# intellerce/controlanimate

Measured on AMD Instinct MI355X. Metric: frames_per_sec, higher is better.
Workload: dtype fp16

## Files before the change

controlanimate_amd/_build.py:

```python
from __future__ import annotations

import os
import subprocess
import sys
from concurrent.futures import ThreadPoolExecutor

CSRC = os.path.join(os.path.dirname(os.path.abspath(__file__)), "csrc")
LIB = os.path.join(CSRC, "libcontrolanimate_hip.so")
SOURCES = ["ca_gemm.hip", "ca_gemm_pp.hip", "ca_gemm_ar.hip", "ca_norm.hip", "ca_attention.hip", "ca_elementwise.hip", "ca_upscale.hip", "ca_color.hip", "ca_canny.hip"]
HEADERS = ["ca_common.h", "ca_gemm_core.h", "ca_gemm_pp2.h", "ca_gemm_wres.h", "ca_gemm_ps.h", "ca_gemm_pq.h", "ca_gemm_ar.h", "ca_ff_fused.h", "ca_attn_out.h", "ca_tattn_fused.h", "ca_xattn_fused.h", "ca_gemm_seq.h", "ca_conv_wino.h", os.path.join("..", "..", "include", "controlanimate_hip.h")]
FLAGS = ["--offload-arch=gfx950", "-O3", "-std=c++17", "-fPIC", "-Wall", "-Wno-unused-function",
         "-mllvm", "-amdgpu-mfma-vgpr-form"]


EXTRA = {"ca_attention.hip": ["-fno-honor-nans"],
         "ca_color.hip": ["-ffp-contract=off"]}


def _extra_env_flags() -> list:
    return os.environ.get("CA_HIPCC_FLAGS", "").split()


def _hipcc() -> str:
    for cand in (os.environ.get("HIPCC"), "/opt/rocm/bin/hipcc", "hipcc"):
        if cand and (os.path.sep not in cand or os.path.exists(cand)):
            return cand
    raise RuntimeError("hipcc not found")


def _stale(out: str, deps: list[str]) -> bool:
    if not os.path.exists(out):
        return True
    t = os.path.getmtime(out)
    return any(os.path.getmtime(d) > t for d in deps)


LIB_EXP = os.path.join(CSRC, "libcontrolanimate_hip_exp.so")
LIB_STAMPS = os.path.join(CSRC, "libcontrolanimate_hip_stamps.so")


def build(force: bool = False, verbose: bool = True, experiments: bool = False, stamps: bool = False) -> str:
    hipcc = _hipcc()
# ... 35 lines not shown
```

controlanimate_amd/_capi.py:

```python
from __future__ import annotations

import ctypes as C
import os

_HERE = os.path.dirname(os.path.abspath(__file__))
LIB_PATH = os.environ.get("CA_HIP_LIB") or os.path.join(_HERE, "csrc", "libcontrolanimate_hip.so")

CA_BF16, CA_F16 = 0, 1
CA_F32 = 2
CA_ACT_NONE, CA_ACT_SILU = 0, 1
ABI_VERSION = 16


class CAHipUnavailable(RuntimeError):
    pass


class CAHipError(RuntimeError):
    pass


class GemmArgs(C.Structure):
    _fields_ = [
        ("a", C.c_void_p), ("a2", C.c_void_p), ("w", C.c_void_p), ("c", C.c_void_p),
# ... 155 lines not shown
    "ca_latents_to_nhwc": (C.c_int, [C.c_void_p, C.c_void_p, C.c_int32, C.c_int32, C.c_int32, C.c_int32, C.c_int32,
                                      C.c_int32, C.c_int32, C.c_float, C.c_int32, C.c_void_p]),
    "ca_nhwc_to_ncfhw_f32": (C.c_int, [C.c_void_p, C.c_void_p, C.c_int32, C.c_int32, C.c_int32, C.c_int32, C.c_int32,
                                        C.c_int32, C.c_int32, C.c_int32, C.c_void_p]),
    "ca_ncfhw_to_nhwc": (C.c_int, [C.c_void_p, C.c_int32, C.POINTER(C.c_int64), C.c_void_p, C.c_int32, C.c_int32,
                                    C.c_int32, C.c_int32, C.c_int32, C.c_int32, C.c_int32, C.c_void_p]),
    "ca_cfg_scheduler_step": (C.c_int, [C.c_void_p, C.c_int32, C.c_int32, C.c_float, C.c_void_p, C.c_void_p,
                                         C.c_void_p, C.c_void_p, C.c_int32, C.c_int32, C.c_int32, C.c_int32,
                                         C.POINTER(C.c_float), C.c_float, C.c_void_p]),
    "ca_lincomb": (C.c_int, [C.c_void_p, C.POINTER(C.c_void_p), C.POINTER(C.c_float), C.c_int32, C.c_int64, C.c_void_p]),
    "ca_conv3x3_narrow": (C.c_int, [C.POINTER(ConvNarrowArgs), C.c_void_p]),
    "ca_conv3x3_narrow_plan_name": (C.c_int, [C.POINTER(ConvNarrowArgs), C.c_char_p, C.c_int32]),
    "ca_rgb8_to_nhwc": (C.c_int, [C.c_void_p, C.c_void_p, C.c_int32, C.c_int32, C.c_int32, C.c_int32, C.c_void_p]),
    "ca_resize_lanczos4_u8": (C.c_int, [C.c_void_p, C.c_void_p, C.c_int32, C.c_int32, C.c_int32, C.c_int32, C.c_int32,
                                         C.c_void_p, C.c_void_p, C.c_void_p, C.c_void_p, C.c_void_p]),
    "ca_color_match_workspace_bytes": (C.c_int64, [C.c_int32, C.c_int64]),
    "ca_hist_u8x3": (C.c_int, [C.c_void_p, C.c_void_p, C.c_int32, C.c_int64, C.c_void_p]),
    "ca_color_moments_f64": (C.c_int, [C.c_void_p, C.c_void_p, C.c_void_p, C.c_void_p, C.c_int32, C.c_int64, C.c_void_p, C.c_int64, C.c_void_p]),
    "ca_color_transform_f64": (C.c_int, [C.c_void_p, C.c_void_p, C.c_void_p, C.c_void_p, C.c_void_p, C.c_void_p, C.c_int32, C.c_int64, C.c_void_p]),
    "ca_sort_f64_segments": (C.c_int, [C.c_void_p, C.c_void_p, C.c_int32, C.c_int64, C.c_void_p, C.c_int64, C.c_void_p]),
    "ca_color_rank_map_f64": (C.c_int, [C.c_void_p, C.c_void_p, C.c_void_p, C.c_void_p, C.c_void_p, C.c_void_p, C.c_int32, C.c_int64,
                                         C.c_void_p, C.c_int64, C.c_void_p]),
    "ca_color_finish_u8": (C.c_int, [C.c_void_p, C.c_void_p, C.c_int32, C.c_int64, C.c_int32, C.c_void_p, C.c_int64, C.c_void_p]),
    "ca_canny_workspace_bytes": (C.c_int64, [C.c_int32, C.c_int32, C.c_int32]),
    "ca_canny_tile_w": (C.c_int32, []),
    "ca_canny_tile_h": (C.c_int32, []),
    "ca_canny_classify": (C.c_int, [C.c_void_p, C.c_int32, C.c_int32, C.c_int32, C.c_int32, C.c_int32, C.c_int32, C.c_void_p, C.c_int64, C.c_void_p]),
    "ca_canny_link": (C.c_int, [C.c_int32, C.c_int32, C.c_int32, C.c_void_p, C.c_int64, C.c_void_p]),
    "ca_canny_link_stage": (C.c_int, [C.c_int32, C.c_int32, C.c_int32, C.c_void_p, C.c_int64, C.c_int32, C.c_void_p]),
    "ca_canny_emit": (C.c_int, [C.c_int32, C.c_int32, C.c_int32, C.c_void_p, C.c_int64, C.c_void_p, C.c_void_p, C.c_int32, C.c_int32, C.c_void_p]),
    "ca_conv_up2_phase_supported": (C.c_int, [C.POINTER(ConvArgs)]),
    "ca_conv_up2_phase": (C.c_int, [C.POINTER(ConvArgs), C.c_void_p]),
    "ca_conv_up2_phase_plan_name": (C.c_int, [C.POINTER(ConvArgs), C.c_char_p, C.c_int32]),
}

_lib = None


def lib() -> C.CDLL:
    global _lib
    if _lib is not None:
        return _lib
    import torch
    if not os.path.exists(LIB_PATH):
        raise CAHipUnavailable(
            f"{LIB_PATH} is missing: the HIP extension is not built. Run "
            "`python -m controlanimate_amd._build` (needs hipcc); there is no CPU fallback.")
    try:
        handle = C.CDLL(LIB_PATH)
    except OSError as e:
        raise CAHipUnavailable(f"cannot load {LIB_PATH}: {e}") from e
    for name, (res, args) in SYMBOLS.items():
        fn = getattr(handle, name)
        fn.restype = res
        fn.argtypes = args
    if handle.ca_abi_version() != ABI_VERSION:
        raise CAHipUnavailable(f"ABI mismatch: library {handle.ca_abi_version()} vs binding {ABI_VERSION}; rebuild")
    _lib = handle
    return handle


def check(rc: int, what: str) -> None:
    if rc != 0:
        msg = lib().ca_last_error()
        raise CAHipError(f"{what} failed with code {rc}: {msg.decode() if msg else ''}")
```

controlanimate_amd/context.py:

```python
from __future__ import annotations

from dataclasses import dataclass, field
from typing import Optional

import torch


@dataclass
class ExecCtx:
    b: int
    f: int
    dtype: torch.dtype
    temb: torch.Tensor
    emb_groups: int
    ehs: Optional[torch.Tensor] = None
    frames_per_kv: int = 1
    kv_mod: int = 0
    gn_frames_per_stat: int = 1
    cache: dict = field(default_factory=dict)

    @property
    def images(self) -> int:
        return self.b * self.f

    def rows_per_emb_group(self, h: int, w: int) -> int:
        return self.images // self.emb_groups * h * w


class Dispatch:
    gemm_ar = True
    ff_fused = True
    tattn_fused = True
    xattn_fused = True
    attn_out_fused = True
    xattn_ip_fused = True
    conv_winograd = True
    gn_winograd = True
    conv_up2_phase = True
    ln_row_sums = True
    repeat_kernel = True
    ln_fold = True
    cfg_shared = True
    cn_cfg_dedup = True
    controlnet_streams = 2


dispatch = Dispatch()
```

controlanimate_amd/controlnet.py:

```python
from __future__ import annotations

import dataclasses
from collections import OrderedDict

from typing import List, Optional, Sequence, Tuple, Union

import torch
from torch import nn

from . import kernels as K
from .context import ExecCtx
from .layers import HipConv1x1, HipConv3x3
from .unet import FrozenConfig, HipModelMixin, TimestepEmbedding, Timesteps
from .unet_blocks import UNetMidBlock3DCrossAttn, get_down_block


class ControlNetConditioningEmbedding(nn.Module):
    def __init__(self, conditioning_embedding_channels: int, conditioning_channels: int = 3,
                 block_out_channels: Tuple[int, ...] = (16, 32, 96, 256)):
        super().__init__()
        self.conv_in = HipConv3x3(conditioning_channels, block_out_channels[0])
        blocks = []
        for i in range(len(block_out_channels) - 1):
            blocks.append(HipConv3x3(block_out_channels[i], block_out_channels[i]))
            blocks.append(HipConv3x3(block_out_channels[i], block_out_channels[i + 1], stride=2))
        self.blocks = nn.ModuleList(blocks)
        self.conv_out = HipConv3x3(block_out_channels[-1], conditioning_embedding_channels)
        nn.init.zeros_(self.conv_out.weight)

    def pack(self, arena, dtype):
        self.conv_in.pack(arena, dtype)
        for b in self.blocks:
            b.pack(arena, dtype)
        self.conv_out.pack(arena, dtype)

    def forward(self, cond_nhwc: torch.Tensor) -> torch.Tensor:
        e = self.conv_in.run(cond_nhwc, act=K.ACT_SILU)
        for b in self.blocks:
            e = b.run(e, act=K.ACT_SILU)
        return self.conv_out.run(e)


class ControlNetModel(HipModelMixin, nn.Module):
    def __init__(self, in_channels: int = 4, conditioning_channels: int = 3, flip_sin_to_cos: bool = True, freq_shift: int = 0,
                 down_block_types: Tuple[str, ...] = ("CrossAttnDownBlock2D", "CrossAttnDownBlock2D", "CrossAttnDownBlock2D", "DownBlock2D"),
                 only_cross_attention: bool = False, block_out_channels: Tuple[int, ...] = (320, 640, 1280, 1280),
                 layers_per_block: int = 2, downsample_padding: int = 1, mid_block_scale_factor: float = 1, act_fn: str = "silu",
                 norm_num_groups: int = 32, norm_eps: float = 1e-5, cross_attention_dim: int = 768,
                 attention_head_dim: Union[int, Tuple[int, ...]] = 8, use_linear_projection: bool = False,
                 conditioning_embedding_out_channels: Tuple[int, ...] = (16, 32, 96, 256), global_pool_conditions: bool = False,
                 **unused):
        super().__init__()
        self._init_exec()
        if use_linear_projection or global_pool_conditions:
            raise NotImplementedError("not part of the SD1.5 ControlNet configuration")
        cfg = dict(locals())
        for k in ("self", "unused", "__class__"):
            cfg.pop(k, None)
        self.config = FrozenConfig(cfg)
        time_embed_dim = block_out_channels[0] * 4
        self.conv_in = HipConv3x3(in_channels, block_out_channels[0])
        self.time_proj = Timesteps(block_out_channels[0], flip_sin_to_cos, freq_shift)
        self.time_embedding = TimestepEmbedding(block_out_channels[0], time_embed_dim, act_fn=act_fn)
        self.controlnet_cond_embedding = ControlNetConditioningEmbedding(block_out_channels[0], conditioning_channels,
                                                                         conditioning_embedding_out_channels)
        self.down_blocks = nn.ModuleList([])
        self.controlnet_down_blocks = nn.ModuleList([HipConv1x1(block_out_channels[0], block_out_channels[0])])
        if isinstance(attention_head_dim, int):
            attention_head_dim = (attention_head_dim,) * len(down_block_types)
        common = dict(temb_channels=time_embed_dim, resnet_eps=norm_eps, resnet_groups=norm_num_groups,
                      cross_attention_dim=cross_attention_dim, use_inflated_groupnorm=True, use_motion_module=False)
        output_channel = block_out_channels[0]
        for i, t in enumerate(down_block_types):
            input_channel, output_channel = output_channel, block_out_channels[i]
            is_final = i == len(block_out_channels) - 1
            self.down_blocks.append(get_down_block(t, num_layers=layers_per_block, in_channels=input_channel,
                                                   out_channels=output_channel, add_downsample=not is_final,
                                                   attn_num_head_channels=attention_head_dim[i], **common))
            for _ in range(layers_per_block + (0 if is_final else 1)):
                self.controlnet_down_blocks.append(HipConv1x1(output_channel, output_channel))
        self.controlnet_mid_block = HipConv1x1(block_out_channels[-1], block_out_channels[-1])
        self.mid_block = UNetMidBlock3DCrossAttn(in_channels=block_out_channels[-1], output_scale_factor=mid_block_scale_factor,
                                                 attn_num_head_channels=attention_head_dim[-1], **common)
        for m in list(self.controlnet_down_blocks) + [self.controlnet_mid_block]:
            nn.init.zeros_(m.weight)
        self._hints: "OrderedDict[int, dict]" = OrderedDict()

    @classmethod
    def from_config(cls, config: dict, **kwargs):
        merged = {k: v for k, v in dict(config).items() if not k.startswith("_")}
        merged.update(kwargs)
        return cls(**merged)

    def hint_slot(self, controlnet_cond: Optional[torch.Tensor] = None) -> Optional[dict]:
# ... 207 lines not shown
```

controlanimate_amd/kernels.py:

```python
from __future__ import annotations

import ctypes as C
from typing import Optional

import torch

from . import _capi
from .context import dispatch
from ._capi import (AttnArgs, ConvArgs, ConvNarrowArgs, FfArgs, TattnArgs, XattnArgs, GemmArgs, GroupNormArgs, LayerNormArgs, CA_ACT_NONE,
                    CA_ACT_SILU, CA_BF16, CA_F16, check, lib)

ACT_NONE, ACT_SILU = CA_ACT_NONE, CA_ACT_SILU
ACT_QUICK_GELU, ACT_GELU = 2, 3


def dt_code(dtype: torch.dtype) -> int:
    if dtype == torch.bfloat16:
        return CA_BF16
    if dtype == torch.float16:
        return CA_F16
    raise TypeError(f"activations must be bf16 or fp16, got {dtype}")


def _stream() -> int:
# ... 200 lines not shown
        return None
    if _plan_sink is not None:
        _plan_sink.append(("xattn_ip_out128" if kv_frag_ip is not None else "xattn_out128") if w_out_frag is not None else "xattn_fused128")
    check(lib().ca_xattn_fused(C.byref(args), _stream()), "ca_xattn_fused")
    return o


def row_sums_of(t: torch.Tensor):
    return getattr(t, "_row_sums", None)


def carry_row_sums(dst: torch.Tensor, src: torch.Tensor) -> torch.Tensor:
    s = getattr(src, "_row_sums", None)
    if s is not None:
        dst._row_sums = s
    return dst


class RowStats:

    def __init__(self, x: torch.Tensor, eps: float = 1e-5, sums=None):
        self.x, self.eps, self._t, self.sums = x, float(eps), None, sums

    def tensor(self) -> torch.Tensor:
        if self._t is None:
            self._t = row_stats(self.x, self.eps)
        return self._t


def conv3x3(x: torch.Tensor, w: torch.Tensor, *, x2: Optional[torch.Tensor] = None,
            bias: Optional[torch.Tensor] = None, rowbias: Optional[torch.Tensor] = None,
            rows_per_group: int = 0, residual: Optional[torch.Tensor] = None, stride: int = 1,
            upsample: bool = False, alpha: float = 1.0, post_scale: float = 1.0, act: int = ACT_NONE,
            out_f32: bool = False, pad_asym: bool = False, w_wino: Optional[torch.Tensor] = None) -> torch.Tensor:
    _req_cuda(x, w, x2, bias, rowbias, residual, w_wino)
    assert x.dim() == 4 and x.is_contiguous() and w.dim() == 4 and w.is_contiguous()
    images, hin, win, cin1 = x.shape
    cin2 = 0
    if x2 is not None:
        assert x2.is_contiguous() and x2.shape[:3] == x.shape[:3] and x2.dtype == x.dtype
        cin2 = x2.shape[3]
    cout = w.shape[0]
    assert tuple(w.shape[1:]) == (3, 3, cin1 + cin2) and w.dtype == x.dtype
    hl, wl = (hin * 2, win * 2) if upsample else (hin, win)
    pad = 1 if pad_asym else 2
    hout, wout = (hl + pad - 3) // stride + 1, (wl + pad - 3) // stride + 1
    y = torch.empty((images, hout, wout, cout), device=x.device, dtype=torch.float32 if out_f32 else x.dtype)
    ld_res = 0
    if residual is not None:
        assert residual.dtype == x.dtype and residual.is_contiguous() and residual.numel() == images * hout * wout * cout, \
            f"residual {tuple(residual.shape)} {residual.dtype} contiguous={residual.is_contiguous()} vs output {(images, hout, wout, cout)} {x.dtype}"
        ld_res = cout
    if rowbias is not None:
        assert rowbias.dtype == torch.float32 and rowbias.dim() == 2 and rowbias.shape[1] == cout and rows_per_group > 0
    if bias is not None:
        assert bias.dtype == torch.float32 and bias.numel() == cout
    args = ConvArgs(x=_p(x), x2=_p(x2), w=_p(w), y=_p(y), bias=_p(bias), rowbias=_p(rowbias),
                    residual=_p(residual), ld_res=ld_res,
                    ld_rowbias=rowbias.stride(0) if rowbias is not None else 0, images=images, hin=hin,
                    win=win, cin1=cin1, cin2=cin2, cout=cout, stride=stride, upsample=int(upsample),
                    rows_per_group=rows_per_group, alpha=alpha, post_scale=post_scale, act=act,
                    out_f32=int(out_f32), dtype=dt_code(x.dtype), pad_asym=int(pad_asym))
    if w_wino is not None and dispatch.conv_winograd:
        assert w_wino.dtype == x.dtype and w_wino.is_contiguous() and tuple(w_wino.shape) == (16, cout, cin1 + cin2)
        args.w_wino = _p(w_wino)
    wbytes = int(lib().ca_conv3x3_workspace_bytes(C.byref(args)))
    if wbytes > 0:
        ws = torch.empty((wbytes,), device=x.device, dtype=torch.uint8)
        args.workspace, args.workspace_bytes = _p(ws), wbytes
    _record_plan(lib().ca_conv3x3_plan_name, args)
    check(lib().ca_conv3x3(C.byref(args), _stream()), "ca_conv3x3")
    return y


def _up2_args(x, w_phase, bias, residual, alpha, y=None) -> ConvArgs:
    images, hin, win, cin = x.shape
    cout = w_phase.shape[1]
    return ConvArgs(x=_p(x), w=_p(w_phase), y=_p(y) if y is not None else _p(x), bias=_p(bias), residual=_p(residual),
                    ld_res=cout if residual is not None else 0, images=images, hin=hin, win=win, cin1=cin, cin2=0, cout=cout, stride=1,
                    upsample=1, rows_per_group=0, alpha=alpha, post_scale=1.0, act=ACT_NONE, out_f32=0, dtype=dt_code(x.dtype), pad_asym=0)


def conv_up2_phase_supported(x: torch.Tensor, w_phase: torch.Tensor, *, bias: Optional[torch.Tensor] = None,
                             residual: Optional[torch.Tensor] = None, alpha: float = 1.0) -> bool:
    if x.dim() != 4 or w_phase.dim() != 5 or not x.is_contiguous() or x.dtype not in (torch.float16, torch.bfloat16):
        return False
    return bool(lib().ca_conv_up2_phase_supported(C.byref(_up2_args(x, w_phase, bias, residual, alpha))))


def conv_up2_phase(x: torch.Tensor, w_phase: torch.Tensor, *, bias: Optional[torch.Tensor] = None,
                   residual: Optional[torch.Tensor] = None, alpha: float = 1.0) -> torch.Tensor:
    _req_cuda(x, w_phase, bias, residual)
    assert x.dim() == 4 and x.is_contiguous() and w_phase.dim() == 5 and w_phase.is_contiguous() and w_phase.dtype == x.dtype
    images, hin, win, cin = x.shape
    cout = w_phase.shape[1]
# ... 473 lines not shown
```

controlanimate_amd/layers.py:

```python
from __future__ import annotations

from typing import Callable, List, Optional, Sequence, Tuple

import torch
from torch import nn

from . import kernels as K
from .context import dispatch

ALIGN = 256


class Packed:

    __slots__ = ("shape", "dtype", "fill", "offset", "t", "frag")

    def __init__(self, shape, dtype, fill):
        self.shape = tuple(int(s) for s in shape)
        self.dtype = dtype
        self.fill = fill
        self.offset = -1
        self.t: Optional[torch.Tensor] = None
        self.frag = None

# ... 120 lines not shown
        super().__init__()
        self.in_channels, self.out_channels = in_channels, out_channels
        self.weight = nn.Parameter(torch.empty(out_channels, in_channels, 1, 1))
        self.bias = nn.Parameter(torch.zeros(out_channels))
        nn.init.normal_(self.weight, std=in_channels ** -0.5)
        self.w = self.b = None

    def pack(self, arena: WeightArena, dtype):
        self.w = arena.add((self.out_channels, self.in_channels), dtype, lambda: _f32(self.weight).reshape(self.out_channels, self.in_channels))
        self.b = arena.add((self.out_channels,), torch.float32, lambda: _f32(self.bias))

    def run(self, a: torch.Tensor, **kw) -> torch.Tensor:
        return K.gemm(a, self.w.t, bias=self.b.t, **kw)


def phase_weights(w: torch.Tensor) -> torch.Tensor:
    sel = torch.tensor([[[1.0, 0.0, 0.0], [0.0, 1.0, 1.0]], [[1.0, 1.0, 0.0], [0.0, 0.0, 1.0]]], dtype=w.dtype, device=w.device)
    wp = torch.einsum("ydk,xel,oikl->yxodei", sel, sel, w)
    return wp.reshape(4, w.shape[0], 2, 2, w.shape[1]).contiguous()


class HipConv3x3(nn.Module):

    def __init__(self, in_channels: int, out_channels: int, stride: int = 1):
        super().__init__()
        self.in_channels, self.out_channels, self.stride = in_channels, out_channels, stride
        self.cin_pad = (in_channels + 7) // 8 * 8
        self.weight = nn.Parameter(torch.empty(out_channels, in_channels, 3, 3))
        self.bias = nn.Parameter(torch.zeros(out_channels))
        nn.init.normal_(self.weight, std=(9 * in_channels) ** -0.5)
        self.w = self.b = None
        self.winograd = True
        self.up2_phase = False

    def _packed_weight(self) -> torch.Tensor:
        w = _f32(self.weight).permute(0, 2, 3, 1)
        if self.cin_pad != self.in_channels:
            w = torch.nn.functional.pad(w, (0, self.cin_pad - self.in_channels))
        return w.contiguous()

    def _winograd_weight(self) -> torch.Tensor:
        g = torch.tensor([[1.0, 0.0, 0.0], [0.5, 0.5, 0.5], [0.5, -0.5, 0.5], [0.0, 0.0, 1.0]], dtype=torch.float32, device=self.weight.device)
        u = torch.einsum("xk,oikl,yl->xyoi", g, _f32(self.weight), g)
        return u.reshape(16, self.out_channels, self.in_channels).contiguous()

    def pack(self, arena: WeightArena, dtype):
        self.w = arena.add((self.out_channels, 3, 3, self.cin_pad), dtype, self._packed_weight)
        self.b = arena.add((self.out_channels,), torch.float32, lambda: _f32(self.bias))
        self.u = None
        if (dispatch.conv_winograd and self.stride == 1 and self.winograd and self.in_channels >= 640 and self.in_channels % 64 == 0
                and self.out_channels % 320 == 0):
            self.u = arena.add((16, self.out_channels, self.in_channels), dtype, self._winograd_weight)
        self.wp = None
        if dispatch.conv_up2_phase and self.up2_phase and self.stride == 1 and self.in_channels % 64 == 0 and self.out_channels % 320 == 0:
            self.wp = arena.add((4, self.out_channels, 2, 2, self.in_channels), dtype, lambda: phase_weights(_f32(self.weight)))

    def run(self, x: torch.Tensor, **kw) -> torch.Tensor:
        wp = getattr(self, "wp", None)
        if wp is not None and dispatch.conv_up2_phase and kw.get("upsample") and set(kw) <= {"upsample", "residual", "alpha"}:
            ph = {k: v for k, v in kw.items() if k != "upsample"}
            if K.conv_up2_phase_supported(x, wp.t, bias=self.b.t, **ph):
                return K.conv_up2_phase(x, wp.t, bias=self.b.t, **ph)
        u = getattr(self, "u", None)
        return K.conv3x3(x, self.w.t, bias=self.b.t, stride=self.stride, w_wino=None if u is None else u.t, **kw)


class HipGroupNorm(nn.Module):
    def __init__(self, num_groups: int, num_channels: int, eps: float = 1e-5):
        super().__init__()
        self.num_groups, self.num_channels, self.eps = num_groups, num_channels, eps
        self.weight = nn.Parameter(torch.ones(num_channels))
        self.bias = nn.Parameter(torch.zeros(num_channels))
        self.g = self.b = None

    def pack(self, arena: WeightArena, dtype):
        self.g = arena.add((self.num_channels,), torch.float32, lambda: _f32(self.weight))
        self.b = arena.add((self.num_channels,), torch.float32, lambda: _f32(self.bias))

    def run(self, x: torch.Tensor, *, x2: Optional[torch.Tensor] = None, frames_per_stat: int = 1, act: int = K.ACT_NONE):
        return K.group_norm(x, self.g.t, self.b.t, x2=x2, groups=self.num_groups, frames_per_stat=frames_per_stat,
                            eps=self.eps, act=act)


class HipLayerNorm(nn.Module):
    def __init__(self, dim: int, eps: float = 1e-5):
        super().__init__()
        self.dim, self.eps = dim, eps
        self.weight = nn.Parameter(torch.ones(dim))
        self.bias = nn.Parameter(torch.zeros(dim))
        self.g = self.b = None

    def pack(self, arena: WeightArena, dtype):
        self.g = arena.add((self.dim,), torch.float32, lambda: _f32(self.weight))
        self.b = arena.add((self.dim,), torch.float32, lambda: _f32(self.bias))

    def run(self, x: torch.Tensor, *, pos: Optional[torch.Tensor] = None, rows_per_frame: int = 1, frames: int = 1):
        return K.layer_norm(x, self.g.t, self.b.t, pos=pos, rows_per_frame=rows_per_frame, frames=frames, eps=self.eps)
# ... 62 lines not shown
```

controlanimate_amd/unet.py:

```python
from __future__ import annotations

from collections import OrderedDict

import dataclasses
import json
import os
from dataclasses import dataclass
from typing import Any, Dict, Optional, Tuple, Union

import torch
from torch import nn

from . import kernels as K
from .context import ExecCtx, dispatch
from .layers import HipGroupNorm, HipLinear, WeightArena, pack_concat_bias, pack_concat_rows
from .resnet import InflatedConv3d, InflatedGroupNorm, ResnetBlock3D
from .unet_blocks import UNetMidBlock3DCrossAttn, get_down_block, get_up_block


@dataclass
class UNet3DConditionOutput:
    sample: torch.Tensor


# ... 246 lines not shown
        class_embed_type: Optional[str] = None,
        num_class_embeds: Optional[int] = None,
        upcast_attention: bool = False,
        resnet_time_scale_shift: str = "default",
        use_inflated_groupnorm: bool = False,
        time_cond_proj_dim: Optional[int] = None,
        use_motion_module: bool = False,
        motion_module_resolutions: Tuple[int, ...] = (1, 2, 4, 8),
        motion_module_mid_block: bool = False,
        motion_module_decoder_only: bool = False,
        motion_module_type: Optional[str] = None,
        motion_module_kwargs: Optional[dict] = None,
        unet_use_cross_frame_attention: Optional[bool] = None,
        unet_use_temporal_attention: Optional[bool] = None,
        **unused,
    ):
        super().__init__()
        self._init_exec()
        if class_embed_type is not None or num_class_embeds is not None or dual_cross_attention or use_linear_projection:
            raise NotImplementedError("not part of the SD1.5 configuration the reference runs")
        if act_fn not in ("silu", "swish") or resnet_time_scale_shift != "default" or center_input_sample:
            raise NotImplementedError("SD1.5 uses silu / default time-embedding norm")
        cfg = dict(locals())
        for k in ("self", "unused", "__class__"):
            cfg.pop(k, None)
        cfg.update(unused)
        self.config = FrozenConfig(cfg)
        self.sample_size = sample_size
        self.in_channels = in_channels
        motion_module_kwargs = dict(motion_module_kwargs or {})
        time_embed_dim = block_out_channels[0] * 4

        self.conv_in = InflatedConv3d(in_channels, block_out_channels[0])
        self.time_proj = Timesteps(block_out_channels[0], flip_sin_to_cos, freq_shift)
        self.time_embedding = TimestepEmbedding(block_out_channels[0], time_embed_dim, act_fn=act_fn, cond_proj_dim=time_cond_proj_dim)

        self.down_blocks = nn.ModuleList([])
        self.up_blocks = nn.ModuleList([])
        if isinstance(attention_head_dim, int):
            attention_head_dim = (attention_head_dim,) * len(down_block_types)
        common = dict(temb_channels=time_embed_dim, resnet_eps=norm_eps, resnet_groups=norm_num_groups,
                      cross_attention_dim=cross_attention_dim, use_inflated_groupnorm=use_inflated_groupnorm,
                      motion_module_type=motion_module_type, motion_module_kwargs=motion_module_kwargs,
                      unet_use_cross_frame_attention=bool(unet_use_cross_frame_attention),
                      unet_use_temporal_attention=bool(unet_use_temporal_attention))
        output_channel = block_out_channels[0]
        for i, t in enumerate(down_block_types):
            res = 2 ** i
            input_channel, output_channel = output_channel, block_out_channels[i]
            self.down_blocks.append(get_down_block(
                t, num_layers=layers_per_block, in_channels=input_channel, out_channels=output_channel,
                add_downsample=i != len(block_out_channels) - 1, attn_num_head_channels=attention_head_dim[i],
                use_motion_module=use_motion_module and (res in motion_module_resolutions) and not motion_module_decoder_only,
                **common))
        if mid_block_type != "UNetMidBlock3DCrossAttn":
            raise ValueError(f"unknown mid_block_type : {mid_block_type}")
        mid = UNetMidBlock3DCrossAttn(in_channels=block_out_channels[-1], output_scale_factor=mid_block_scale_factor,
                                      attn_num_head_channels=attention_head_dim[-1],
                                      use_motion_module=use_motion_module and motion_module_mid_block, **common)
        self.num_upsamplers = 0
        rev = list(reversed(block_out_channels))
        rev_heads = list(reversed(attention_head_dim))
        output_channel = rev[0]
        for i, t in enumerate(up_block_types):
            res = 2 ** (3 - i)
            is_final = i == len(block_out_channels) - 1
            prev_output_channel, output_channel = output_channel, rev[i]
            input_channel = rev[min(i + 1, len(block_out_channels) - 1)]
            if not is_final:
                self.num_upsamplers += 1
            self.up_blocks.append(get_up_block(
                t, num_layers=layers_per_block + 1, in_channels=input_channel, out_channels=output_channel,
                prev_output_channel=prev_output_channel, add_upsample=not is_final, attn_num_head_channels=rev_heads[i],
                use_motion_module=use_motion_module and (res in motion_module_resolutions), **common))
        self.mid_block = mid
        self.conv_norm_out = InflatedGroupNorm(norm_num_groups, block_out_channels[0], norm_eps)
        self.conv_act = nn.SiLU()
        self.conv_out = InflatedConv3d(block_out_channels[0], out_channels)

    def _to_nhwc(self, t: torch.Tensor, device, cpad: Optional[int] = None) -> torch.Tensor:
        b, c, f, h, w = t.shape
        cpad = cpad or c
        want = (f * h * w * c, 1, h * w * c, w * c, c)
        if (t.is_cuda and t.dtype == self.act_dtype and cpad == c
                and all(n == 1 or s == e for n, s, e in zip(t.shape, t.stride(), want))):
            return t.permute(0, 2, 3, 4, 1).reshape(b * f, h, w, c)
        return K.ncfhw_to_nhwc(t.to(device), cpad, self.act_dtype)

    @torch.no_grad()
    def forward_nhwc(self, x: torch.Tensor, b: int, f: int, timestep, encoder_hidden_states: torch.Tensor,
                     down_residuals=None, mid_residual=None, timestep_cond=None, cfg_identical_halves: bool = False) -> torch.Tensor:
        device = x.device
        self._ensure_ready(device)
        _, h, w, _ = x.shape
        if any(s % (2 ** self.num_upsamplers) for s in (h, w)):
            raise NotImplementedError("latent height/width must be multiples of 8 (vid2vid.py floors frames to /64)")
        ehs, cache = self._prompt(encoder_hidden_states, device)
        if ehs.shape[0] != b:
            raise ValueError(f"encoder_hidden_states batch {ehs.shape[0]} != sample batch {b}")
        temb = self._time_embedding(timestep, b, device, timestep_cond)
        ctx = ExecCtx(b=b, f=f, dtype=self.act_dtype, temb=temb, emb_groups=b, ehs=ehs, frames_per_kv=f,
                      gn_frames_per_stat=1 if self.config.use_inflated_groupnorm else f, cache=cache)
        first = self.down_blocks[0]
        shared = (cfg_identical_halves and dispatch.cfg_shared and b == 2 and getattr(first, "has_cross_attention", False) and
                  (not torch.is_tensor(timestep) or timestep.numel() == 1) and (timestep_cond is None or timestep_cond.shape[0] == 1))
        if shared:
            half_ctx = dataclasses.replace(ctx, b=1, temb=temb[:1], emb_groups=1)
            xh = self.conv_in.run(x[: x.shape[0] // 2])
            skips = [K.repeat_batch(xh)]
            x, outs = first(xh, ctx, half_ctx=half_ctx)
            skips += outs
# ... 94 lines not shown
```

include/controlanimate_hip.h:

```cpp
#ifndef CONTROLANIMATE_HIP_H
#define CONTROLANIMATE_HIP_H

#include <stdint.h>

#ifdef __cplusplus
extern "C" {
#endif

#define CA_ABI_VERSION 16

#define CA_BF16 0
#define CA_F16 1
#define CA_F32 2

#define CA_OK 0
#define CA_ERR_INVALID_ARG (-1)
#define CA_ERR_UNSUPPORTED (-2)
#define CA_ERR_LAUNCH (-3)

#define CA_ACT_NONE 0
#define CA_ACT_SILU 1
#define CA_ACT_QUICK_GELU 2
#define CA_ACT_GELU 3

// ... 102 lines not shown
int ca_ln_finish_sums(const float* sums, int parts, int64_t rows, int k, float eps, float* mean_rstd, void* stream);
int ca_gemm_plan_name(const ca_gemm_args* args, char* buf, int32_t len);

typedef struct ca_conv_args {
  const void* x;
  const void* x2;
  const void* w;
  void* y;
  const float* bias;
  const float* rowbias;
  const void* residual;
  int64_t ld_res, ld_rowbias;
  int32_t images, hin, win, cin1, cin2, cout;
  int32_t stride;
  int32_t upsample;
  int32_t rows_per_group;
  float alpha, post_scale;
  int32_t act;
  int32_t out_f32;
  int32_t dtype;
  void* workspace;
  int64_t workspace_bytes;
  int32_t pad_asym;
  const void* w_wino;
  int32_t x_is_wino_v;
} ca_conv_args;
int ca_pack_w_wino(const void* w, int32_t cout, int32_t cin, int32_t dtype, void* dst, void* stream);
int64_t ca_conv3x3_workspace_bytes(const ca_conv_args* args);
int ca_conv3x3(const ca_conv_args* args, void* stream);
int ca_conv3x3_plan_name(const ca_conv_args* args, char* buf, int32_t len);
int ca_conv_up2_phase_supported(const ca_conv_args* args);
int ca_conv_up2_phase(const ca_conv_args* args, void* stream);
int ca_conv_up2_phase_plan_name(const ca_conv_args* args, char* buf, int32_t len);

typedef struct ca_groupnorm_args {
  const void* x;
  const void* x2;
  void* y;
  const float* gamma;
  const float* beta;
  float* partials;
  int32_t images, hw, c1, c2;
  int32_t groups;
  int32_t frames_per_stat;
  float eps;
  int32_t act;
  int32_t dtype;
  void* wino_v;
  int32_t wino_h, wino_w;
} ca_groupnorm_args;
int ca_groupnorm_wino_supported(const ca_groupnorm_args* args);
int64_t ca_groupnorm_partials_floats(int32_t images, int32_t hw, int32_t frames_per_stat, int32_t groups);
int ca_groupnorm_stats(const ca_groupnorm_args* args, void* stream);
int ca_groupnorm_apply(const ca_groupnorm_args* args, void* stream);
int ca_groupnorm(const ca_groupnorm_args* args, void* stream);

typedef struct ca_layernorm_args {
  const void* x; void* y;
  const float* gamma; const float* beta;
  const float* pos;
  int64_t rows;
  int32_t c;
  int32_t rows_per_frame, frames;
  float eps;
  int32_t dtype;
  float* stats;
// ... 122 lines not shown
```

Baseline: 16.30.

## Add specialized few-channel 3x3 conv kernels for conv_in, conv_out and ControlNet embedding

Adds a new HIP source with two kernel families for 3x3 convolutions whose channel counts are small. One targets cin=8 to cout=320 (the UNet/ControlNet conv_in) and keeps the whole weight in shared memory. The other is a thin-N MFMA kernel for cout<=96 (conv_out and the conditioning embedding blocks), replacing the general GEMM/Winograd paths that pad poorly on these shapes. The new path is selected through per-layer flags and dispatch toggles, and any case outside its shape and alignment checks falls back to the old path.

```diff
diff --git a/controlanimate_amd/_build.py b/controlanimate_amd/_build.py
--- a/controlanimate_amd/_build.py
+++ b/controlanimate_amd/_build.py
@@ -7,7 +7,7 @@
 
 CSRC = os.path.join(os.path.dirname(os.path.abspath(__file__)), "csrc")
 LIB = os.path.join(CSRC, "libcontrolanimate_hip.so")
-SOURCES = ["ca_gemm.hip", "ca_gemm_pp.hip", "ca_gemm_ar.hip", "ca_norm.hip", "ca_attention.hip", "ca_elementwise.hip", "ca_upscale.hip", "ca_color.hip", "ca_canny.hip"]
+SOURCES = ["ca_gemm.hip", "ca_gemm_pp.hip", "ca_gemm_ar.hip", "ca_norm.hip", "ca_attention.hip", "ca_elementwise.hip", "ca_upscale.hip", "ca_conv_thin.hip", "ca_color.hip", "ca_canny.hip"]
 HEADERS = ["ca_common.h", "ca_gemm_core.h", "ca_gemm_pp2.h", "ca_gemm_wres.h", "ca_gemm_ps.h", "ca_gemm_pq.h", "ca_gemm_ar.h", "ca_ff_fused.h", "ca_attn_out.h", "ca_tattn_fused.h", "ca_xattn_fused.h", "ca_gemm_seq.h", "ca_conv_wino.h", os.path.join("..", "..", "include", "controlanimate_hip.h")]
 FLAGS = ["--offload-arch=gfx950", "-O3", "-std=c++17", "-fPIC", "-Wall", "-Wno-unused-function",
          "-mllvm", "-amdgpu-mfma-vgpr-form"]
diff --git a/controlanimate_amd/_capi.py b/controlanimate_amd/_capi.py
--- a/controlanimate_amd/_capi.py
+++ b/controlanimate_amd/_capi.py
@@ -211,6 +211,9 @@
     "ca_conv_up2_phase_supported": (C.c_int, [C.POINTER(ConvArgs)]),
     "ca_conv_up2_phase": (C.c_int, [C.POINTER(ConvArgs), C.c_void_p]),
     "ca_conv_up2_phase_plan_name": (C.c_int, [C.POINTER(ConvArgs), C.c_char_p, C.c_int32]),
+    "ca_conv3x3_thin_supported": (C.c_int, [C.POINTER(ConvArgs)]),
+    "ca_conv3x3_thin": (C.c_int, [C.POINTER(ConvArgs), C.c_void_p]),
+    "ca_conv3x3_thin_plan_name": (C.c_int, [C.POINTER(ConvArgs), C.c_char_p, C.c_int32]),
 }
 
 _lib = None
diff --git a/controlanimate_amd/context.py b/controlanimate_amd/context.py
--- a/controlanimate_amd/context.py
+++ b/controlanimate_amd/context.py
@@ -37,6 +37,8 @@
     conv_winograd = True
     gn_winograd = True
     conv_up2_phase = True
+    conv_in_strip = True
+    conv_thin = True
     ln_row_sums = True
     repeat_kernel = True
     ln_fold = True
diff --git a/controlanimate_amd/controlnet.py b/controlanimate_amd/controlnet.py
--- a/controlanimate_amd/controlnet.py
+++ b/controlanimate_amd/controlnet.py
@@ -27,6 +27,8 @@
         self.blocks = nn.ModuleList(blocks)
         self.conv_out = HipConv3x3(block_out_channels[-1], conditioning_embedding_channels)
         nn.init.zeros_(self.conv_out.weight)
+        for m in (self.conv_in, *self.blocks):
+            m.thin = True
 
     def pack(self, arena, dtype):
         self.conv_in.pack(arena, dtype)
@@ -60,6 +62,7 @@
         self.config = FrozenConfig(cfg)
         time_embed_dim = block_out_channels[0] * 4
         self.conv_in = HipConv3x3(in_channels, block_out_channels[0])
+        self.conv_in.thin = True
         self.time_proj = Timesteps(block_out_channels[0], flip_sin_to_cos, freq_shift)
         self.time_embedding = TimestepEmbedding(block_out_channels[0], time_embed_dim, act_fn=act_fn)
         self.controlnet_cond_embedding = ControlNetConditioningEmbedding(block_out_channels[0], conditioning_channels,
diff --git a/controlanimate_amd/csrc/ca_conv_thin.hip b/controlanimate_amd/csrc/ca_conv_thin.hip
--- /dev/null
+++ b/controlanimate_amd/csrc/ca_conv_thin.hip
@@ -0,0 +1,270 @@
+#include "ca_common.h"
+
+namespace {
+
+__device__ __forceinline__ void pixel_of(int p, int hout, int wout, int& img, int& oy, int& ox) {
+  if (p < 0) {
+    img = 0, oy = -(1 << 20), ox = -(1 << 20);
+    return;
+  }
+  const int hw = hout * wout;
+  img = p / hw;
+  const int r = p - img * hw;
+  oy = r / wout;
+  ox = r - oy * wout;
+}
+
+template <int DT>
+__device__ __forceinline__ void epilogue4(f32x4 acc, float* v, const float* __restrict__ bias, const u16* res, int64_t ld_res, int p, int c,
+                                          float alpha, float post, int act) {
+  float b[4] = {0.f, 0.f, 0.f, 0.f};
+  if (bias) {
+    const f32x4 q = *reinterpret_cast<const f32x4*>(bias + c);
+#pragma unroll
+    for (int r = 0; r < 4; ++r) b[r] = q[r];
+  }
+#pragma unroll
+  for (int r = 0; r < 4; ++r) v[r] = (acc[r] + b[r]) * alpha;
+  if (res) {
+    const u32x2 q = *reinterpret_cast<const u32x2*>(res + (int64_t)p * ld_res + c);
+#pragma unroll
+    for (int r = 0; r < 4; ++r) v[r] += Elem<DT>::to_f((u16)(q[r >> 1] >> ((r & 1) * 16)));
+  }
+#pragma unroll
+  for (int r = 0; r < 4; ++r) v[r] = act_f(v[r] * post, act);
+}
+
+constexpr int IN_COUT = 320, IN_K = 72;
+template <int DT, int MT>
+__global__ __launch_bounds__(256) void k_conv_in(const u16* __restrict__ x, const u16* __restrict__ w, u16* __restrict__ y,
+                                                 const float* __restrict__ bias, const u16* res, int64_t ld_res, int hin, int win, int npix,
+                                                 float alpha, float post, int act) {
+  __shared__ __attribute__((aligned(16))) u16 ws[IN_COUT * IN_K];
+  const int lane = threadIdx.x & 63, wave = threadIdx.x >> 6;
+  const int col = lane & 15, g = lane >> 4;
+  for (int i = threadIdx.x; i < IN_COUT * IN_K / 8; i += 256) st16(ws + i * 8, ld16(w + i * 8));
+
+  const int tile0 = (blockIdx.x * 4 + wave) * (MT * 16);
+  u32x4 b[3][MT];
+#pragma unroll
+  for (int m = 0; m < MT; ++m) {
+    int p = tile0 + m * 16 + col, img, oy, ox;
+    if (p >= npix) p = -1;
+    pixel_of(p, hin, win, img, oy, ox);
+#pragma unroll
+    for (int j = 0; j < 3; ++j) {
+      const int tap = 4 * j + g;
+      const int ky = tap / 3, kx = tap - ky * 3;
+      const int iy = oy + ky - 1, ix = ox + kx - 1;
+      const bool ok = tap < 9 && iy >= 0 && iy < hin && ix >= 0 && ix < win;
+      b[j][m] = ok ? ld16(x + (int64_t)((img * hin + iy) * win + ix) * 8) : (u32x4){0u, 0u, 0u, 0u};
+    }
+  }
+  __syncthreads();
+
+  const int rsub = 8 * (col >> 2) + (col & 3);
+  for (int t = 0; t < IN_COUT / 32; ++t) {
+    u32x4 a[2][3];
+#pragma unroll
+    for (int h = 0; h < 2; ++h)
+#pragma unroll
+      for (int j = 0; j < 3; ++j) {
+        const int tap = 4 * j + g;
+        a[h][j] = tap < 9 ? ld16(ws + (32 * t + rsub + 4 * h) * IN_K + tap * 8) : (u32x4){0u, 0u, 0u, 0u};
+      }
+#pragma unroll
+    for (int m = 0; m < MT; ++m) {
+      f32x4 acc[2];
+#pragma unroll
+      for (int h = 0; h < 2; ++h) {
+        acc[h] = (f32x4){0.f, 0.f, 0.f, 0.f};
+#pragma unroll
+        for (int j = 0; j < 3; ++j) acc[h] = Elem<DT>::mfma(a[h][j], b[j][m], acc[h]);
+      }
+      const int p = tile0 + m * 16 + col;
+      if (p >= npix) continue;
+      const int c = 32 * t + 8 * g;
+      float v[8];
+      epilogue4<DT>(acc[0], v, bias, res, ld_res, p, c, alpha, post, act);
+      epilogue4<DT>(acc[1], v + 4, bias, res, ld_res, p, c + 4, alpha, post, act);
+      st16(y + (int64_t)p * IN_COUT + c, pack8<DT>(v));
+    }
+  }
+}
+
+template <int DT, int NT, int MT>
+__global__ __launch_bounds__(256) void k_conv_thin(const u16* __restrict__ x, const u16* __restrict__ w, void* y,
+                                                   const float* __restrict__ bias, const u16* res, int64_t ld_res, int hin, int win,
+                                                   int hout, int wout, int cin, int cout, int npix, int stride, float alpha, float post,
+                                                   int act, int out_f32) {
+  const int lane = threadIdx.x & 63, wave = threadIdx.x >> 6;
+  const int col = lane & 15, kq = (lane >> 4) * 8;
+  const int tile0 = (blockIdx.x * 4 + wave) * (MT * 16);
+  if (tile0 >= npix) return;
+  int iy0[MT], ix0[MT], img[MT];
+#pragma unroll
+  for (int m = 0; m < MT; ++m) {
+    int p = tile0 + m * 16 + col, oy, ox;
+    if (p >= npix) p = -1;
+    pixel_of(p, hout, wout, img[m], oy, ox);
+    iy0[m] = oy * stride - 1, ix0[m] = ox * stride - 1;
+  }
+  f32x4 acc[NT][MT];
+#pragma unroll
+  for (int n = 0; n < NT; ++n)
+#pragma unroll
+    for (int m = 0; m < MT; ++m) acc[n][m] = (f32x4){0.f, 0.f, 0.f, 0.f};
+
+  const int ktot = 9 * cin;
+  const u16* wrow[NT];
+  bool wok[NT];
+#pragma unroll
+  for (int n = 0; n < NT; ++n) {
+    wok[n] = n * 16 + col < cout;
+    wrow[n] = w + (int64_t)min(n * 16 + col, cout - 1) * ktot;
+  }
+  const u32x4 zero = {0u, 0u, 0u, 0u};
+
+  if (cin % 32 == 0) {
+    for (int tap = 0; tap < 9; ++tap) {
+      const int ky = tap / 3, kx = tap - ky * 3;
+      int64_t off[MT];
+#pragma unroll
+      for (int m = 0; m < MT; ++m) {
+        const int iy = iy0[m] + ky, ix = ix0[m] + kx;
+        const bool ok = iy >= 0 && iy < hin && ix >= 0 && ix < win;
+        off[m] = ok ? (int64_t)((img[m] * hin + iy) * win + ix) * cin + kq : -1;
+      }
+      for (int c0 = 0; c0 < cin; c0 += 32) {
+        u32x4 a[NT], b[MT];
+#pragma unroll
+        for (int n = 0; n < NT; ++n) a[n] = wok[n] ? ld16(wrow[n] + tap * cin + c0 + kq) : zero;
+#pragma unroll
+        for (int m = 0; m < MT; ++m) b[m] = off[m] >= 0 ? ld16(x + off[m] + c0) : zero;
+#pragma unroll
+        for (int n = 0; n < NT; ++n)
+#pragma unroll
+          for (int m = 0; m < MT; ++m) acc[n][m] = Elem<DT>::mfma(a[n], b[m], acc[n][m]);
+      }
+    }
+  } else {
+    for (int k0 = 0; k0 < ktot; k0 += 32) {
+      const int kk = k0 + kq;
+      const bool kok = kk < ktot;
+      const int tap = kok ? kk / cin : 0, c = kk - tap * cin;
+      const int ky = tap / 3, kx = tap - ky * 3;
+      u32x4 a[NT], b[MT];
+#pragma unroll
+      for (int n = 0; n < NT; ++n) a[n] = (kok && wok[n]) ? ld16(wrow[n] + kk) : zero;
+#pragma unroll
+      for (int m = 0; m < MT; ++m) {
+        const int iy = iy0[m] + ky, ix = ix0[m] + kx;
+        const bool ok = kok && iy >= 0 && iy < hin && ix >= 0 && ix < win;
+        b[m] = ok ? ld16(x + (int64_t)((img[m] * hin + iy) * win + ix) * cin + c) : zero;
+      }
+#pragma unroll
+      for (int n = 0; n < NT; ++n)
+#pragma unroll
+        for (int m = 0; m < MT; ++m) acc[n][m] = Elem<DT>::mfma(a[n], b[m], acc[n][m]);
+    }
+  }
+
+  const int cq = (lane >> 4) * 4;
+#pragma unroll
+  for (int m = 0; m < MT; ++m) {
+    const int p = tile0 + m * 16 + col;
+    if (p >= npix) continue;
+#pragma unroll
+    for (int n = 0; n < NT; ++n) {
+      const int c = n * 16 + cq;
+      if (c >= cout) continue;
+      float v[4];
+      epilogue4<DT>(acc[n][m], v, bias, res, ld_res, p, c, alpha, post, act);
+      if (out_f32) {
+        *reinterpret_cast<f32x4*>(reinterpret_cast<float*>(y) + (int64_t)p * cout + c) = (f32x4){v[0], v[1], v[2], v[3]};
+      } else {
+        u32x2 o;
+        o[0] = pack2<DT>(v[0], v[1]);
+        o[1] = pack2<DT>(v[2], v[3]);
+        *reinterpret_cast<u32x2*>(reinterpret_cast<u16*>(y) + (int64_t)p * cout + c) = o;
+      }
+    }
+  }
+}
+
+enum ThinPlan { TP_NONE = 0, TP_IN320, TP_N16, TP_N32, TP_N96 };
+constexpr int IN_MT = 2;
+
+struct ThinShape {
+  int hout, wout, npix;
+};
+
+ThinPlan thin_capable(const ca_conv_args* a, ThinShape* s) {
+  if (!a || !a->x || !a->w || !a->y || a->x2 || a->cin2 != 0 || a->images <= 0 || a->hin <= 0 || a->win <= 0) return TP_NONE;
+  if (a->upsample || a->pad_asym || a->x_is_wino_v || a->rowbias || (a->stride != 1 && a->stride != 2)) return TP_NONE;
+  if (a->dtype != CA_F16 && a->dtype != CA_BF16) return TP_NONE;
+  if (a->act != CA_ACT_NONE && a->act != CA_ACT_SILU) return TP_NONE;
+  if (a->cin1 <= 0 || a->cout <= 0 || a->cout % 4 != 0) return TP_NONE;
+  if ((((uintptr_t)a->x | (uintptr_t)a->w | (uintptr_t)a->y | (uintptr_t)a->residual | (uintptr_t)a->bias) & 15) != 0) return TP_NONE;
+  if (a->residual && (a->ld_res < a->cout || a->ld_res % 4 != 0)) return TP_NONE;
+  const int hout = (a->hin - 1) / a->stride + 1, wout = (a->win - 1) / a->stride + 1;
+  const int64_t npix = (int64_t)a->images * hout * wout, nin = (int64_t)a->images * a->hin * a->win;
+  if (npix + 1024 >= ((int64_t)1 << 31) || nin >= ((int64_t)1 << 31)) return TP_NONE;
+  s->hout = hout, s->wout = wout, s->npix = (int)npix;
+  if (a->cout == IN_COUT) return (a->cin1 == 8 && a->stride == 1 && !a->out_f32) ? TP_IN320 : TP_NONE;
+  if (a->cout > 96 || !(a->cin1 % 32 == 0 || a->cin1 == 8 || a->cin1 == 16)) return TP_NONE;
+  return a->cout <= 16 ? TP_N16 : a->cout <= 32 ? TP_N32 : TP_N96;
+}
+
+bool thin_pays(const ca_conv_args* a, ThinPlan plan, const ThinShape& s) {
+  (void)a, (void)plan, (void)s;
+  return true;
+}
+
+template <int DT, int NT, int MT>
+void launch_thin(const ca_conv_args* a, const ThinShape& s, hipStream_t st) {
+  hipLaunchKernelGGL((k_conv_thin<DT, NT, MT>), dim3(ceil_div_i(s.npix, 4 * MT * 16)), dim3(256), 0, st, (const u16*)a->x, (const u16*)a->w,
+                     a->y, a->bias, (const u16*)a->residual, (int64_t)a->ld_res, a->hin, a->win, s.hout, s.wout, a->cin1, a->cout, s.npix,
+                     a->stride, a->alpha, a->post_scale, a->act, a->out_f32);
+}
+
+template <int DT>
+void launch_thin_dt(const ca_conv_args* a, ThinPlan plan, const ThinShape& s, hipStream_t st) {
+  if (plan == TP_IN320)
+    hipLaunchKernelGGL((k_conv_in<DT, IN_MT>), dim3(ceil_div_i(s.npix, 4 * IN_MT * 16)), dim3(256), 0, st, (const u16*)a->x,
+                       (const u16*)a->w, (u16*)a->y, a->bias, (const u16*)a->residual, (int64_t)a->ld_res, a->hin, a->win, s.npix, a->alpha,
+                       a->post_scale, a->act);
+  else if (plan == TP_N16) launch_thin<DT, 1, 8>(a, s, st);
+  else if (plan == TP_N32) launch_thin<DT, 2, 8>(a, s, st);
+  else launch_thin<DT, 6, 4>(a, s, st);
+}
+
+}
+
+extern "C" int ca_conv3x3_thin_supported(const ca_conv_args* a) {
+  ThinShape s{};
+  const ThinPlan plan = thin_capable(a, &s);
+  return plan != TP_NONE && thin_pays(a, plan, s) ? 1 : 0;
+}
+
+extern "C" int ca_conv3x3_thin(const ca_conv_args* a, void* stream) {
+  ThinShape s{};
+  const ThinPlan plan = thin_capable(a, &s);
+  CA_REQUIRE(plan != TP_NONE, "ca_conv3x3_thin: arguments the few-channel kernels do not take (one fp16 / bf16 source, stride 1 or 2, padding 1, no "
+             "upsampling / row bias, activation none or SiLU, 16-byte aligned operands, and cin = 8 with cout = 320, or cout %% 4 == 0, cout <= 96 with "
+             "cin %% 32 == 0 or cin = 8 / 16)");
+  hipStream_t st = (hipStream_t)stream;
+  if (a->dtype == CA_F16) launch_thin_dt<CA_F16>(a, plan, s, st);
+  else launch_thin_dt<CA_BF16>(a, plan, s, st);
+  CA_CHECK_LAUNCH("ca_conv3x3_thin");
+  return CA_OK;
+}
+
+extern "C" int ca_conv3x3_thin_plan_name(const ca_conv_args* a, char* buf, int32_t len) {
+  CA_REQUIRE(buf && len > 0, "ca_conv3x3_thin_plan_name: buffer");
+  ThinShape s{};
+  const ThinPlan plan = thin_capable(a, &s);
+  CA_REQUIRE(plan != TP_NONE, "ca_conv3x3_thin_plan_name: arguments the few-channel kernels do not take");
+  snprintf(buf, (size_t)len, "%s", plan == TP_IN320 ? "thin_in320" : plan == TP_N16 ? "thin_n16m128" : plan == TP_N32 ? "thin_n32m128" : "thin_n96m64");
+  return CA_OK;
+}
diff --git a/controlanimate_amd/kernels.py b/controlanimate_amd/kernels.py
--- a/controlanimate_amd/kernels.py
+++ b/controlanimate_amd/kernels.py
@@ -256,7 +256,7 @@
             bias: Optional[torch.Tensor] = None, rowbias: Optional[torch.Tensor] = None,
             rows_per_group: int = 0, residual: Optional[torch.Tensor] = None, stride: int = 1,
             upsample: bool = False, alpha: float = 1.0, post_scale: float = 1.0, act: int = ACT_NONE,
-            out_f32: bool = False, pad_asym: bool = False, w_wino: Optional[torch.Tensor] = None) -> torch.Tensor:
+            out_f32: bool = False, pad_asym: bool = False, w_wino: Optional[torch.Tensor] = None, thin: bool = False) -> torch.Tensor:
     _req_cuda(x, w, x2, bias, rowbias, residual, w_wino)
     assert x.dim() == 4 and x.is_contiguous() and w.dim() == 4 and w.is_contiguous()
     images, hin, win, cin1 = x.shape
@@ -285,6 +285,10 @@
                     win=win, cin1=cin1, cin2=cin2, cout=cout, stride=stride, upsample=int(upsample),
                     rows_per_group=rows_per_group, alpha=alpha, post_scale=post_scale, act=act,
                     out_f32=int(out_f32), dtype=dt_code(x.dtype), pad_asym=int(pad_asym))
+    if thin and lib().ca_conv3x3_thin_supported(C.byref(args)):
+        _record_plan(lib().ca_conv3x3_thin_plan_name, args)
+        check(lib().ca_conv3x3_thin(C.byref(args), _stream()), "ca_conv3x3_thin")
+        return y
     if w_wino is not None and dispatch.conv_winograd:
         assert w_wino.dtype == x.dtype and w_wino.is_contiguous() and tuple(w_wino.shape) == (16, cout, cin1 + cin2)
         args.w_wino = _p(w_wino)
diff --git a/controlanimate_amd/layers.py b/controlanimate_amd/layers.py
--- a/controlanimate_amd/layers.py
+++ b/controlanimate_amd/layers.py
@@ -176,6 +176,7 @@
         self.w = self.b = None
         self.winograd = True
         self.up2_phase = False
+        self.thin = False
 
     def _packed_weight(self) -> torch.Tensor:
         w = _f32(self.weight).permute(0, 2, 3, 1)
@@ -206,7 +207,8 @@
             if K.conv_up2_phase_supported(x, wp.t, bias=self.b.t, **ph):
                 return K.conv_up2_phase(x, wp.t, bias=self.b.t, **ph)
         u = getattr(self, "u", None)
-        return K.conv3x3(x, self.w.t, bias=self.b.t, stride=self.stride, w_wino=None if u is None else u.t, **kw)
+        thin = self.thin and (dispatch.conv_in_strip if self.out_channels == 320 else dispatch.conv_thin)
+        return K.conv3x3(x, self.w.t, bias=self.b.t, stride=self.stride, w_wino=None if u is None else u.t, thin=bool(thin), **kw)
 
 
 class HipGroupNorm(nn.Module):
diff --git a/controlanimate_amd/unet.py b/controlanimate_amd/unet.py
--- a/controlanimate_amd/unet.py
+++ b/controlanimate_amd/unet.py
@@ -302,6 +302,7 @@
         time_embed_dim = block_out_channels[0] * 4
 
         self.conv_in = InflatedConv3d(in_channels, block_out_channels[0])
+        self.conv_in.thin = True
         self.time_proj = Timesteps(block_out_channels[0], flip_sin_to_cos, freq_shift)
         self.time_embedding = TimestepEmbedding(block_out_channels[0], time_embed_dim, act_fn=act_fn, cond_proj_dim=time_cond_proj_dim)
 
@@ -347,6 +348,7 @@
         self.conv_norm_out = InflatedGroupNorm(norm_num_groups, block_out_channels[0], norm_eps)
         self.conv_act = nn.SiLU()
         self.conv_out = InflatedConv3d(block_out_channels[0], out_channels)
+        self.conv_out.thin = True
 
     def _to_nhwc(self, t: torch.Tensor, device, cpad: Optional[int] = None) -> torch.Tensor:
         b, c, f, h, w = t.shape
diff --git a/include/controlanimate_hip.h b/include/controlanimate_hip.h
--- a/include/controlanimate_hip.h
+++ b/include/controlanimate_hip.h
@@ -158,6 +158,9 @@
 int ca_conv_up2_phase_supported(const ca_conv_args* args);
 int ca_conv_up2_phase(const ca_conv_args* args, void* stream);
 int ca_conv_up2_phase_plan_name(const ca_conv_args* args, char* buf, int32_t len);
+int ca_conv3x3_thin_supported(const ca_conv_args* args);
+int ca_conv3x3_thin(const ca_conv_args* args, void* stream);
+int ca_conv3x3_thin_plan_name(const ca_conv_args* args, char* buf, int32_t len);
 
 typedef struct ca_groupnorm_args {
   const void* x;
```

Result: no change. 16.30 (-0.0%).
